# prajwaljpj/GUAVA_renderer

Measured on AMD Instinct MI355X. Metric: rendered frames/sec @512x512, ~100k Gaussians, higher is better.
Workload: dtype f32; 1 GPU; guava-avatar-synth-100k-512-deform+raster; pipeline=EHM LBS -> Gaussian assembly -> rasterize, gaussians=100000, channels=32, global_batch=32, parallelism=frame-sharded x1, batches_in_flight=4, placement=shared, exp=exact-poly, colour_accum=f32 mfma (bit-exact)

## Files before the change

### guava_renderer_amd/csrc/deform.hip

```cpp
#include <climits>
#include <cstdlib>
#include <string>

#include "../../include/gsr.h"
#include "../../include/gsr_deform.h"
#include "deform_internal.h"
#include "gsr_internal.h"
#include "preprocess_dev.h"

namespace gsr {

#ifndef GSR_DEFORM_NOSTORE
#define GSR_DEFORM_NOSTORE 0
#endif

constexpr int kLbsFrames = 16;
constexpr int kLbsSplit = 4;
constexpr int kLbsSplit1 = 16;

struct Parents {
    int8_t p[GSR_LBS_MAX_JOINTS];
};

__device__ __forceinline__ void rodrigues_one(const float* __restrict__ pose, int t, int pose2rot, float (&R)[9]) {
// ... 275 lines not shown
    if (NB > 0) blend_tiled_mfma_part(as, betas, NB, sd_tiled, NB, t, bA, bok, w, hi, lane, NW);
    if (NP > 0 && v_posed) blend_tiled_mfma_part(ap, feat, NP, pd_tiled, NP, t, bA, bok, w, hi, lane, NW);
#pragma unroll
    for (int r = 0; r < 16; r++) {
        red[w][0][r][lane] = as[r];
        red[w][1][r][lane] = ap[r];
    }
    __syncthreads();
#pragma unroll
    for (int i = 0; i < 16 / NW; i++) {
        const int r = (16 / NW) * w + i;
        const int b = b0 + (r & 3) + 8 * (r >> 2) + 4 * hi;
        if (!mok || b >= B) continue;
        float S = red[0][0][r][lane], Pz = red[0][1][r][lane];
#pragma unroll
        for (int u = 1; u < NW; u++) { S += red[u][0][r][lane]; Pz += red[u][1][r][lane]; }
        const float tv = vt[(int64_t)b * vt_stride + m];
        const float vs = NB > 0 ? tv + S : tv;
        v_shaped[(int64_t)b * M + m] = vs;
        if (v_posed) v_posed[(int64_t)b * M + m] = Pz + vs;
    }
}

__device__ __forceinline__ float blend_tiled_one(const float* __restrict__ coef, const float4* __restrict__ tb,
                                                 int K, int t, int w, int hi, int lane) {
    const int nkg = (K + 7) / 8;
    const float4* __restrict__ p = tb + (int64_t)t * nkg * 64 + lane;
    float acc = 0.f;
    for (int g0 = w; g0 < nkg; g0 += 4 * kTiledUnroll) {
        float4 v[kTiledUnroll];
        float a[kTiledUnroll][4];
#pragma unroll
        for (int u = 0; u < kTiledUnroll; u++) {
            const int g = g0 + 4 * u;
            v[u] = g < nkg ? p[(int64_t)g * 64] : make_float4(0.f, 0.f, 0.f, 0.f);
#pragma unroll
            for (int j = 0; j < 4; j++) {
                const int k = 8 * g + 4 * hi + j;
                a[u][j] = k < K ? coef[k] : 0.f;
            }
        }
#pragma unroll
        for (int u = 0; u < kTiledUnroll; u++) {
            acc = fmaf(a[u][0], v[u].x, acc);
            acc = fmaf(a[u][1], v[u].y, acc);
            acc = fmaf(a[u][2], v[u].z, acc);
// ... 64 lines not shown
static void lbs_blend_attr(size_t lds) {
    static size_t attr = 0;
    if (lds > 65536 && attr < lds) {
        attr = lds;
        hipFuncSetAttribute((const void*)k_lbs_blend<kLbsFrames, kLbsSplit>,
                            hipFuncAttributeMaxDynamicSharedMemorySize, (int)lds);
        hipFuncSetAttribute((const void*)k_lbs_blend<1, kLbsSplit1>, hipFuncAttributeMaxDynamicSharedMemorySize,
                            (int)lds);
    }
}

Blend1Job blend1_job(int M, int NB, int NP, const float* vt, const float* betas, const float* feat, float* vs,
                     float* vp, const GsrLbsSparse* sp, const float* pose, int pose2rot) {
    return Blend1Job{M, NB, vp ? NP : 0, pose2rot, vt, betas, reinterpret_cast<const float4*>(sp->shapedirs_tiled),
                     feat, reinterpret_cast<const float4*>(sp->posedirs_tiled), vs, vp, pose};
}

bool blend_tiled1_applies(int B, int NB, int NP, const float* vp, const GsrLbsSparse* sp) {
    static const bool tiled_on = tune_env("GSR_BLEND_TILED", 1) != 0;
    return B == 1 && tiled_on && sp && (NB == 0 || sp->shapedirs_tiled) && (NP == 0 || !vp || sp->posedirs_tiled) &&
           (NB > 0 || (NP > 0 && vp));
}

static void launch_blend(int B, int M, int NB, int NP, const float* vt, int64_t vt_stride, const float* betas,
                         const float* sd_t, const float* feat, const float* pd, float* vs, float* vp,
                         hipStream_t s, const GsrLbsSparse* sp, const float* pose, int pose2rot) {
    static const bool valu_only = tune_env("GSR_BLEND_VALU", 0) == 1;
    static const bool tiled_on = tune_env("GSR_BLEND_TILED", 1) != 0;
    const bool tiled = tiled_on && sp && (NB == 0 || sp->shapedirs_tiled) &&
                       (NP == 0 || !vp || sp->posedirs_tiled) && (NB > 0 || (NP > 0 && vp));
    if (tiled && B > kLbsFrames && !valu_only) {
        static const int nw_env = tune_env("GSR_BLEND_NW", 0);
        const dim3 grid((M + 31) / 32, (B + 31) / 32);
        const int nw = nw_env == 4 || nw_env == 8 ? nw_env : (grid.x * grid.y <= 512 ? 8 : 4);
        const float4* sdt = reinterpret_cast<const float4*>(sp->shapedirs_tiled);
        const float4* pdt = reinterpret_cast<const float4*>(sp->posedirs_tiled);
        if (nw == 8)
            hipLaunchKernelGGL(k_lbs_blend_tiled<8>, grid, dim3(512), 0, s, B, M, NB, vp ? NP : 0, vt, vt_stride,
                               betas, sdt, feat, pdt, vs, vp);
        else
            hipLaunchKernelGGL(k_lbs_blend_tiled<4>, grid, dim3(256), 0, s, B, M, NB, vp ? NP : 0, vt, vt_stride,
                               betas, sdt, feat, pdt, vs, vp);
        return;
    }
    if (tiled && B == 1) {
        const Blend1Job j = blend1_job(M, NB, NP, vt, betas, feat, vs, vp, sp, pose, pose2rot);
        hipLaunchKernelGGL(k_lbs_blend_tiled1, dim3((M + 31) / 32), dim3(256), 0, s, j);
        return;
    }
    if (B > kLbsFrames && !valu_only) {
        hipLaunchKernelGGL(k_lbs_blend_mfma, dim3((M + 31) / 32, (B + 31) / 32), dim3(256), 0, s, B, M, NB,
                           vp ? NP : 0, vt, vt_stride, betas, sd_t, feat, pd, vs, vp);
        return;
    }
    static const bool single = tune_env("GSR_BLEND_SINGLE", 1) != 0;
    if (B == 1 && single) {
        const size_t lds = lbs_blend_lds(NB, vp ? NP : 0, 1, kLbsSplit1);
// ... 86 lines not shown
        x = fmaf(wv, vs[3 * v], x);
        y = fmaf(wv, vs[3 * v + 1], y);
        z = fmaf(wv, vs[3 * v + 2], z);
    }
#pragma unroll
    for (int off = 32; off > 0; off >>= 1) {
        x += __shfl_xor(x, off);
        y += __shfl_xor(y, off);
        z += __shfl_xor(z, off);
    }
    if (lane < 3) {
        float v = lane == 0 ? x : lane == 1 ? y : z;
        if (joff) v = v + joff[((int64_t)b * J + j) * 3 + lane];
        joints[((int64_t)b * J + j) * 3 + lane] = v;
    }
}

struct ChainJoints {
    const int32_t* row;
    const int32_t* col;
    const float* val;
    const float* vs;
    const float* joff;
};
__global__ __launch_bounds__(16 * GSR_LBS_MAX_JOINTS) void k_lbs_chain(int J, Parents par,
                                                                     const float* __restrict__ rot,
                                                                     float* __restrict__ joints,
                                                                     float* __restrict__ jtrans,
                                                                     float* __restrict__ A,
                                                                     const float* __restrict__ pose, int pose2rot,
                                                                     ChainJoints cj) {
    __shared__ float tm[GSR_LBS_MAX_JOINTS][16];
    __shared__ float ch[GSR_LBS_MAX_JOINTS][16];
    __shared__ int depth[GSR_LBS_MAX_JOINTS];
    __shared__ float sjt[GSR_LBS_MAX_JOINTS * 3];
    __shared__ int maxd;
    const int b = blockIdx.x, t = threadIdx.x;
    const float* Jb = joints + (int64_t)b * J * 3;
    if (cj.row) {
        const int w = t >> 6, lane = t & 63;
        for (int j = w; j < J; j += 16) {
            float x = 0.f, y = 0.f, z = 0.f;
            for (int k = cj.row[j] + lane; k < cj.row[j + 1]; k += 64) {
                const int v = cj.col[k];
                const float wv = cj.val[k];
                x = fmaf(wv, cj.vs[3 * v], x);
                y = fmaf(wv, cj.vs[3 * v + 1], y);
                z = fmaf(wv, cj.vs[3 * v + 2], z);
            }
#pragma unroll
            for (int off = 32; off > 0; off >>= 1) {
                x += __shfl_xor(x, off);
                y += __shfl_xor(y, off);
                z += __shfl_xor(z, off);
            }
            if (lane < 3) {
                float v = lane == 0 ? x : lane == 1 ? y : z;
                if (cj.joff) v = v + cj.joff[j * 3 + lane];
                sjt[3 * j + lane] = v;
                joints[j * 3 + lane] = v;
            }
        }
        __syncthreads();
        Jb = sjt;
    }
    if (t == 0) maxd = 0;
    if (t < J) {
        float R[9];
        if (rot) {
#pragma unroll
            for (int e = 0; e < 9; e++) R[e] = rot[((int64_t)b * J + t) * 9 + e];
        } else {
            rodrigues_one(pose, b * J + t, pose2rot, R);
        }
        float rel[3];
        for (int c = 0; c < 3; c++) rel[c] = t == 0 ? Jb[c] : Jb[3 * t + c] - Jb[3 * par.p[t] + c];
        for (int r = 0; r < 3; r++) {
            for (int c = 0; c < 3; c++) tm[t][4 * r + c] = R[3 * r + c];
            tm[t][4 * r + 3] = rel[r];
        }
        tm[t][12] = 0.f; tm[t][13] = 0.f; tm[t][14] = 0.f; tm[t][15] = 1.f;
        int dd = 0;
        for (int i = t; i > 0 && dd < GSR_LBS_MAX_JOINTS; i = par.p[i]) dd++;
        depth[t] = dd;
    }
// ... 398 lines not shown
        return v >= 1 && v <= 64 ? v : 1;
    }();
    hipLaunchKernelGGL(k_deform_preprocess, dim3(d.nblk, (d.B + fpw - 1) / fpw), dim3(256), 0, s, fpw, dg, d, in,
                       g, o);
}

struct PackTable {
    GsrRowSegment seg[GSR_PACK_MAX_SEGMENTS];
};

__global__ __launch_bounds__(256) void k_pack_rows(PackTable t) {
    const GsrRowSegment sg = t.seg[blockIdx.x];
    const int b = blockIdx.y;
    for (int c = threadIdx.x; c < sg.width; c += 256)
        sg.dst[b * sg.dst_stride + c] = sg.src ? sg.src[b * sg.src_stride + c] : 0.f;
}

namespace {

size_t align256(size_t x) { return (x + 255) & ~(size_t)255; }

struct LbsArena {
    float *rot, *feat, *vs, *vp, *joints, *A;
};

size_t carve_lbs(char* base, int B, int V, int J, LbsArena* a) {
    size_t off = 0;
    auto take = [&](size_t bytes) {
        char* p = base ? base + off : nullptr;
        off += align256(bytes);
        return reinterpret_cast<float*>(p);
    };
    const size_t f = sizeof(float);
    LbsArena t;
    t.rot = take(f * (size_t)B * J * 9);
    t.feat = take(f * (size_t)B * (J > 1 ? J - 1 : 1) * 9);
    t.vs = take(f * (size_t)B * V * 3);
    t.vp = take(f * (size_t)B * V * 3);
    t.joints = take(f * (size_t)B * J * 3);
    t.A = take(f * (size_t)B * J * 16);
    if (a) *a = t;
    return off;
}

int hip_check(const char* what) {
    hipError_t e = hipGetLastError();
    if (e != hipSuccess) return api_fail(GSR_ERR_HIP, (std::string(what) + ": " + hipGetErrorString(e)).c_str());
    return 0;
}

}
}

using namespace gsr;

__global__ __launch_bounds__(256) void k_lbs_tile_base(int K, int M, int64_t n4, const float* __restrict__ base,
                                                       float4* __restrict__ tiled) {
    const int64_t i = (int64_t)blockIdx.x * 256 + threadIdx.x;
    if (i >= n4) return;
    const int nkg = (K + 7) / 8;
    const int lane = (int)(i & 63);
    const int64_t tg = i >> 6;
    const int g = (int)(tg % nkg), t = (int)(tg / nkg);
    const int m = 32 * t + (lane & 31), k0 = 8 * g + 4 * (lane >> 5);
    float v[4];
#pragma unroll
    for (int j = 0; j < 4; j++) v[j] = (m < M && k0 + j < K) ? base[(int64_t)(k0 + j) * M + m] : 0.f;
    tiled[i] = make_float4(v[0], v[1], v[2], v[3]);
}

extern "C" {

size_t gsr_lbs_workspace_bytes(int B, int V, int J, int NB) {
    (void)NB;
    if (B <= 0 || V <= 0 || J <= 0) return 0;
    return carve_lbs(nullptr, B, V, J, nullptr);
}

}

namespace {
void launch_joints(int B, int V, int J, const float* J_regressor, const GsrLbsSparse* sp, const float* vs,
                   const float* joints_offset, float* joints, hipStream_t s) {
    if (sp && sp->jreg_row) {
        hipLaunchKernelGGL(k_lbs_joints_csr, dim3((B * J + 3) / 4), dim3(256), 0, s, B, V, J, sp->jreg_row,
                           sp->jreg_col, sp->jreg_val, vs, joints_offset, joints);
    } else {
        hipLaunchKernelGGL(k_lbs_joints, dim3((J + kJointsPerWG - 1) / kJointsPerWG, B), dim3(256), 0, s, V, J,
                           J_regressor, vs, joints_offset, joints);
    }
}
int check_sparse(const GsrLbsSparse* sp, int J, int NB, int V, const char* who) {
    if (!sp) return 0;
    if (sp->jreg_row && (!sp->jreg_col || !sp->jreg_val))
        return api_fail(GSR_ERR_ARG, (std::string(who) + ": jreg_row without jreg_col / jreg_val").c_str());
    if (sp->skin_k && (sp->skin_k < 0 || sp->skin_k > GSR_LBS_SKIN_MAX_K || !sp->skin_joint || !sp->skin_weight))
        return api_fail(GSR_ERR_ARG, (std::string(who) + ": skin_k must be in [1, 16] with its arrays").c_str());
    if (((uintptr_t)sp->shapedirs_tiled | (uintptr_t)sp->posedirs_tiled) & 15)
        return api_fail(GSR_ERR_ARG, (std::string(who) + ": tiled bases must be 16-byte aligned").c_str());
// ... 10 lines not shown
int gsr_lbs(int B, int V, int J, int NB, const float* v_template, int64_t v_template_stride,
            const float* betas, const float* shapedirs_t, const float* pose, int pose2rot,
            const float* posedirs, const float* J_regressor, const int32_t* parents_host,
            const float* lbs_weights_t, const float* joints_offset, float* verts,
            float* joints_transformed, float* joints, float* vert_transforms,
            float* joint_transforms, float* v_shaped, char* workspace, void* stream) {
    return gsr_lbs_sp(B, V, J, NB, v_template, v_template_stride, betas, shapedirs_t, pose, pose2rot, posedirs,
                      J_regressor, parents_host, lbs_weights_t, joints_offset, verts, joints_transformed, joints,
                      vert_transforms, joint_transforms, v_shaped, workspace, nullptr, stream);
}

int gsr_lbs_sp(int B, int V, int J, int NB, const float* v_template, int64_t v_template_stride,
               const float* betas, const float* shapedirs_t, const float* pose, int pose2rot,
               const float* posedirs, const float* J_regressor, const int32_t* parents_host,
               const float* lbs_weights_t, const float* joints_offset, float* verts,
               float* joints_transformed, float* joints, float* vert_transforms,
               float* joint_transforms, float* v_shaped, char* workspace, const GsrLbsSparse* sp,
               void* stream) {
    return gsr::lbs_run(B, V, J, NB, v_template, v_template_stride, betas, shapedirs_t, pose, pose2rot, posedirs,
                        J_regressor, parents_host, lbs_weights_t, joints_offset, verts, joints_transformed, joints,
                        vert_transforms, joint_transforms, v_shaped, workspace, sp, stream, true);
}

}

int gsr::lbs_run(int B, int V, int J, int NB, const float* v_template, int64_t v_template_stride,
                 const float* betas, const float* shapedirs_t, const float* pose, int pose2rot,
                 const float* posedirs, const float* J_regressor, const int32_t* parents_host,
                 const float* lbs_weights_t, const float* joints_offset, float* verts,
                 float* joints_transformed, float* joints, float* vert_transforms,
                 float* joint_transforms, float* v_shaped, char* workspace, const GsrLbsSparse* sp,
                 void* stream, bool skin, const Blend1Job* companion, bool* companion_done) {
    if (companion_done) *companion_done = false;
    if (B <= 0 || V <= 0) return api_fail(GSR_ERR_ARG, "gsr_lbs: B and V must be positive");
    if (int rc = check_sparse(sp, J, betas ? NB : 0, V, "gsr_lbs")) return rc;
    if (J < 1 || J > GSR_LBS_MAX_JOINTS) return api_fail(GSR_ERR_ARG, "gsr_lbs: J must be in [1, 64]");
    if (!v_template || !pose || !J_regressor || !parents_host || !lbs_weights_t || (skin && !verts) || !workspace)
        return api_fail(GSR_ERR_ARG, "gsr_lbs: null required pointer");
    if (J > 1 && !posedirs) return api_fail(GSR_ERR_ARG, "gsr_lbs: posedirs is null");
    if (v_template_stride != 0 && v_template_stride != (int64_t)V * 3)
        return api_fail(GSR_ERR_ARG, "gsr_lbs: v_template stride must be 0 or V*3");
    if (betas) {
        if (NB <= 0 || !shapedirs_t) return api_fail(GSR_ERR_ARG, "gsr_lbs: betas need NB > 0 and shapedirs");
    } else {
        NB = 0;
    }
    Parents par;
    for (int i = 0; i < GSR_LBS_MAX_JOINTS; i++) par.p[i] = -1;
    if (parents_host[0] != -1) return api_fail(GSR_ERR_ARG, "gsr_lbs: parents[0] must be -1");
    for (int i = 1; i < J; i++) {
        if (parents_host[i] < 0 || parents_host[i] >= i)
            return api_fail(GSR_ERR_ARG, "gsr_lbs: parents must satisfy 0 <= parents[i] < i");
        par.p[i] = (int8_t)parents_host[i];
    }
    hipStream_t s = (hipStream_t)stream;
    LbsArena a;
    carve_lbs(workspace, B, V, J, &a);
    float* vs = v_shaped ? v_shaped : a.vs;
    float* jr = joints ? joints : a.joints;
    float* A = joint_transforms ? joint_transforms : a.A;
    const int NP = (J - 1) * 9;
    const int M = V * 3;

    if (lbs_blend_lds(NB, NP, kLbsFrames, kLbsSplit) > 160 * 1024) return api_fail(GSR_ERR_ARG, "gsr_lbs: NB + 9(J-1) too large for LDS");
    const bool fused = blend_takes_pose(B, NB, NP, a.vp, sp);
    if (!fused) {
        hipLaunchKernelGGL(k_lbs_rodrigues, dim3((B * J + 255) / 256), dim3(256), 0, s, B, J, pose,
                           pose2rot, a.rot, a.feat);
        if (int rc = hip_check("lbs_rodrigues")) return rc;
    }
    if (companion && companion_done && blend_tiled1_applies(B, NB, NP, a.vp, sp)) {
        const Blend1Job ja = blend1_job(M, NB, NP, v_template, betas, a.feat, vs, a.vp, sp, fused ? pose : nullptr,
                                        pose2rot);
        const int na = (M + 31) / 32, nb = (companion->M + 31) / 32;
        hipLaunchKernelGGL(k_lbs_blend_tiled1_pair, dim3(na + nb), dim3(256), 0, s, ja, na, *companion);
        *companion_done = true;
    } else {
        launch_blend(B, M, NB, NP, v_template, v_template_stride, betas, shapedirs_t, a.feat, posedirs, vs, a.vp, s,
                     sp, fused ? pose : nullptr, pose2rot);
    }
    if (int rc = hip_check("lbs_blend")) return rc;
    static const bool chain_joints_on = tune_env("GSR_CHAIN_JOINTS", 1) != 0;
    ChainJoints cj{nullptr, nullptr, nullptr, nullptr, nullptr};
    if (B == 1 && sp && sp->jreg_row && chain_joints_on) {
        cj = ChainJoints{sp->jreg_row, sp->jreg_col, sp->jreg_val, vs, joints_offset};
    } else {
        launch_joints(B, V, J, J_regressor, sp, vs, joints_offset, jr, s);
        if (int rc = hip_check("lbs_joints")) return rc;
    }
    hipLaunchKernelGGL(k_lbs_chain, dim3(B), dim3(16 * GSR_LBS_MAX_JOINTS), 0, s, J, par, fused ? nullptr : a.rot,
                       jr, joints_transformed, A, pose, pose2rot, cj);
    if (int rc = hip_check("lbs_chain")) return rc;
    if (!skin) return 0;
    if (sp && sp->skin_k > 0) {
        const dim3 g((V + 255) / 256, B);
        if (sp->skin_k <= 4)
            hipLaunchKernelGGL(k_lbs_skin_ell<4>, g, dim3(256), 0, s, V, J, sp->skin_k, sp->skin_joint,
                               sp->skin_weight, A, a.vp, verts, vert_transforms);
        else if (sp->skin_k <= 8)
            hipLaunchKernelGGL(k_lbs_skin_ell<8>, g, dim3(256), 0, s, V, J, sp->skin_k, sp->skin_joint,
                               sp->skin_weight, A, a.vp, verts, vert_transforms);
        else
            hipLaunchKernelGGL(k_lbs_skin_ell<16>, g, dim3(256), 0, s, V, J, sp->skin_k, sp->skin_joint,
                               sp->skin_weight, A, a.vp, verts, vert_transforms);
    } else {
        hipLaunchKernelGGL(k_lbs_skin, dim3((V + 255) / 256, B), dim3(256), 0, s, V, J, lbs_weights_t, A,
                           a.vp, verts, vert_transforms);
    }
    return hip_check("lbs_skin");
}

template <int KMAX>
__global__ __launch_bounds__(256) void k_skin_splice(int Vh, int Jh, int K, const int32_t* __restrict__ sj,
                                                     const float* __restrict__ sw, const float* __restrict__ A,
                                                     const float* __restrict__ v_posed, int Vb,
                                                     const int32_t* __restrict__ idx,
                                                     const float* __restrict__ r_eyelid,
                                                     const float* __restrict__ l_eyelid,
                                                     const float* __restrict__ eyelid,
                                                     const float* __restrict__ head_scale,
                                                     const float* __restrict__ hjoints, int hj0, int hj1,
                                                     const float* __restrict__ bjoints, int Jb, int bj0, int bj1,
                                                     float* __restrict__ body, uint32_t* __restrict__ bad) {
    __shared__ float As[GSR_LBS_MAX_JOINTS * 16];
    const int b = blockIdx.y;
    for (int i = threadIdx.x; i < Jh * 16; i += blockDim.x) As[i] = A[(int64_t)b * Jh * 16 + i];
    __syncthreads();
    const int v = blockIdx.x * blockDim.x + threadIdx.x;
    if (v >= Vh) return;
    const int d = idx[v];
    if (d < 0 || d >= Vb) {
// ... 26 lines not shown
        float h = T[4 * c] * px + T[4 * c + 1] * py + T[4 * c + 2] * pz + T[4 * c + 3] * 1.0f;
        if (eyelid) {
            h = h + r_eyelid[3 * v + c] * eyelid[2 * b + 1];
            h = h + l_eyelid[3 * v + c] * eyelid[2 * b];
        }
        if (head_scale) h = h * head_scale[3 * b + c];
        float hs = 0.f, bs = 0.f;
        for (int j = hj0; j < hj1; j++) hs += hjb[3 * j + c];
        for (int j = bj0; j < bj1; j++) bs += bjt[3 * j + c];
        body[((int64_t)b * Vb + d) * 3 + c] = (h - hs / (float)(hj1 - hj0)) + bs / (float)(bj1 - bj0);
    }
}

int gsr::lbs_skin_splice(int B, int Vh, int Jh, const GsrLbsSparse* sp_h, const char* ws_h, int Vb,
                         const int32_t* head_index, const float* r_eyelid, const float* l_eyelid,
                         const float* eyelid, const float* head_scale, const float* head_joints, int hj0, int hj1,
                         const float* body_joints, int Jb, int bj0, int bj1, float* body_v_shaped,
                         uint32_t* bad_index_flag, void* stream) {
    if (!sp_h || sp_h->skin_k <= 0) return 1;
    if (hj0 < 0 || hj1 <= hj0 || hj1 > Jh || bj0 < 0 || bj1 <= bj0 || bj1 > Jb)
        return api_fail(GSR_ERR_ARG, "gsr_ehm_forward: bad reference joint ranges");
    if (eyelid && (!r_eyelid || !l_eyelid)) return api_fail(GSR_ERR_ARG, "gsr_ehm_forward: eyelid bases missing");
    LbsArena a;
    carve_lbs(const_cast<char*>(ws_h), B, Vh, Jh, &a);
    const dim3 g((Vh + 255) / 256, B);
    hipStream_t s = (hipStream_t)stream;
#define GSR_SKS(KM)                                                                                              \
    hipLaunchKernelGGL(k_skin_splice<KM>, g, dim3(256), 0, s, Vh, Jh, sp_h->skin_k, sp_h->skin_joint,            \
                       sp_h->skin_weight, a.A, a.vp, Vb, head_index, r_eyelid, l_eyelid, eyelid, head_scale,     \
                       head_joints, hj0, hj1, body_joints, Jb, bj0, bj1, body_v_shaped, bad_index_flag)
    if (sp_h->skin_k <= 4) GSR_SKS(4);
    else if (sp_h->skin_k <= 8) GSR_SKS(8);
    else GSR_SKS(16);
#undef GSR_SKS
    return hip_check("skin_splice");
}

extern "C" {

int gsr_blend_joints(int B, int V, int J, int NB, const float* v_template, int64_t v_template_stride,
                     const float* betas, const float* shapedirs_t, const float* J_regressor,
                     const float* joints_offset, float* v_shaped, float* joints, void* stream) {
    return gsr_blend_joints_sp(B, V, J, NB, v_template, v_template_stride, betas, shapedirs_t, J_regressor,
                               joints_offset, v_shaped, joints, nullptr, stream);
}

int gsr_blend_joints_sp(int B, int V, int J, int NB, const float* v_template, int64_t v_template_stride,
// ... 123 lines not shown
```

### guava_renderer_amd/csrc/deform_internal.h

```cpp
#pragma once
#include <stdint.h>

#include <hip/hip_runtime.h>

#include "../../include/gsr_deform.h"

namespace gsr {
struct Blend1Job {
    int M, NB, NP, pose2rot;
    const float* vt;
    const float* betas;
    const float4* sd_tiled;
    const float* feat;
    const float4* pd_tiled;
    float* v_shaped;
    float* v_posed;
    const float* pose;
};
bool blend_tiled1_applies(int B, int NB, int NP, const float* vp, const GsrLbsSparse* sp);
Blend1Job blend1_job(int M, int NB, int NP, const float* vt, const float* betas, const float* feat, float* vs,
                     float* vp, const GsrLbsSparse* sp, const float* pose, int pose2rot);
int blend_joints_run(int B, int V, int J, int NB, const float* v_template, int64_t v_template_stride,
                     const float* betas, const float* shapedirs_t, const float* J_regressor,
                     const float* joints_offset, float* v_shaped, float* joints, const GsrLbsSparse* sp,
                     void* stream, bool blend_done);
int lbs_run(int B, int V, int J, int NB, const float* v_template, int64_t v_template_stride, const float* betas,
            const float* shapedirs_t, const float* pose, int pose2rot, const float* posedirs,
            const float* J_regressor, const int32_t* parents_host, const float* lbs_weights_t,
            const float* joints_offset, float* verts, float* joints_transformed, float* joints,
            float* vert_transforms, float* joint_transforms, float* v_shaped, char* workspace,
            const GsrLbsSparse* sp, void* stream, bool skin, const Blend1Job* companion = nullptr,
            bool* companion_done = nullptr);
int lbs_skin_splice(int B, int Vh, int Jh, const GsrLbsSparse* sp_h, const char* ws_h, int Vb,
                    const int32_t* head_index, const float* r_eyelid, const float* l_eyelid, const float* eyelid,
                    const float* head_scale, const float* head_joints, int hj0, int hj1, const float* body_joints,
                    int Jb, int bj0, int bj1, float* body_v_shaped, uint32_t* bad_index_flag, void* stream);
}
```

### guava_renderer_amd/csrc/ehm.hip

```cpp
#include <algorithm>
#include <string>
#include <vector>

#include "../../include/gsr.h"
#include "../../include/gsr_deform.h"
#include "deform_internal.h"
#include "gsr_internal.h"

namespace gsr {
namespace {

constexpr int kEhmMaxSegments = 24;
struct EhmPackTable {
    GsrRowSegment seg[kEhmMaxSegments];
};

__global__ __launch_bounds__(256) void k_ehm_pack(EhmPackTable t) {
    const GsrRowSegment sg = t.seg[blockIdx.x];
    const int b = blockIdx.y;
    for (int c = threadIdx.x; c < sg.width; c += 256)
        sg.dst[b * sg.dst_stride + c] = sg.src ? sg.src[b * sg.src_stride + c] : 0.f;
}

size_t al(size_t x) { return (x + 255) & ~(size_t)255; }

struct EhmArena {
    float *betas_h, *pose_h, *betas_b, *pose_b, *hscale, *eyelid, *joff;
    float *hv, *hj, *vt, *tj;
    char *ws_h, *ws_b;
};

size_t carve_ehm(char* base, const GsrEhm& e, int B, EhmArena* a) {
    size_t off = 0;
    auto take = [&](size_t bytes) {
        char* p = base ? base + off : nullptr;
        off += al(bytes);
        return p;
    };
    auto tf = [&](size_t n) { return reinterpret_cast<float*>(take(sizeof(float) * n)); };
    const size_t b = (size_t)B;
    EhmArena t;
    t.betas_h = tf(b * e.flame.NB);
    t.pose_h = tf(b * 3 * e.flame.J);
    t.betas_b = tf(b * e.body.NB);
    t.pose_b = tf(b * 3 * e.body.J);
    t.hscale = tf(b * 3);
    t.eyelid = tf(b * 2);
    t.joff = tf(b * 3 * e.body.J);
    t.hv = tf(b * e.flame.V * 3);
    t.hj = tf(b * e.flame.J * 3);
    t.vt = tf(b * e.body.V * 3);
    t.tj = tf(b * e.body.J * 3);
    t.ws_h = take(gsr_lbs_workspace_bytes(B, e.flame.V, e.flame.J, e.flame.NB));
    t.ws_b = take(gsr_lbs_workspace_bytes(B, e.body.V, e.body.J, 0));
    if (a) *a = t;
    return off;
}

struct Copy {
    int col, width;
    const float* src;
    int64_t src_stride;
};
int add_block(std::vector<GsrRowSegment>& tab, float* dst, int width, std::vector<Copy> cp, const char* what) {
    std::sort(cp.begin(), cp.end(), [](const Copy& x, const Copy& y) { return x.col < y.col; });
    int c = 0;
    for (const Copy& k : cp) {
        if (k.width <= 0) continue;
        if (k.col < c || k.col + k.width > width)
            return api_fail(GSR_ERR_ARG, (std::string("gsr_ehm_forward: ") + what +
                                          ": a parameter does not fit its coefficient columns").c_str());
        if (k.col > c) tab.push_back(GsrRowSegment{nullptr, dst + c, 0, width, k.col - c, 0});
        tab.push_back(GsrRowSegment{k.src, dst + k.col, k.src_stride, width, k.width, 0});
        c = k.col + k.width;
    }
    if (c < width) tab.push_back(GsrRowSegment{nullptr, dst + c, 0, width, width - c, 0});
    return 0;
// ... 89 lines not shown
    }
    const float* hscale = hsc.p;
    if (hsc.p && !direct(hsc)) {
        tab.push_back(GsrRowSegment{hsc.p, a.hscale, hsc.row_stride, 3, 3, 0});
        hscale = a.hscale;
    }
    const float* joff = jof.p;
    if (jof.p && !direct(jof)) {
        tab.push_back(GsrRowSegment{jof.p, a.joff, jof.row_stride, 3 * Jb, 3 * Jb, 0});
        joff = a.joff;
    }
    if (tab.size() > (size_t)kEhmMaxSegments)
        return api_fail(GSR_ERR_ARG, "gsr_ehm_forward: too many coefficient segments");
    EhmPackTable t;
    for (size_t i = 0; i < tab.size(); i++) {
        if (tab[i].width > 4096) return api_fail(GSR_ERR_ARG, "gsr_ehm_forward: coefficient row too wide");
        t.seg[i] = tab[i];
    }
    hipStream_t s = (hipStream_t)stream;
    hipLaunchKernelGGL(k_ehm_pack, dim3((unsigned)tab.size(), B), dim3(256), 0, s, t);
    if (hipError_t err = hipGetLastError(); err != hipSuccess)
        return api_fail(GSR_ERR_HIP, (std::string("ehm_pack: ") + hipGetErrorString(err)).c_str());

    static const bool skin_splice_on = tune_env("GSR_EHM_SKIN_SPLICE", 1) != 0;
    const bool fuse = skin_splice_on && e.flame.sparse && e.flame.sparse->skin_k > 0;
    Blend1Job body_shape{};
    static const bool pair_on = tune_env("GSR_EHM_PAIR", 1) != 0;
    const bool pair = pair_on && B == 1 && blend_tiled1_applies(1, NBb, 0, nullptr, e.body.sparse);
    if (pair)
        body_shape = blend1_job(Vb * 3, NBb, 0, e.body.v_template, a.betas_b, nullptr, a.vt, nullptr, e.body.sparse,
                                nullptr, 1);
    bool body_blended = false;
    int rc = lbs_run(B, Vh, Jh, NBh, e.flame.v_template, 0, a.betas_h, e.flame.shapedirs_t, a.pose_h, 1,
                     e.flame.posedirs, e.flame.J_regressor, e.flame.parents_host, e.flame.lbs_weights_t, nullptr,
                     a.hv, a.hj, nullptr, nullptr, nullptr, nullptr, a.ws_h, e.flame.sparse, stream, !fuse,
                     pair ? &body_shape : nullptr, &body_blended);
    if (rc) return rc;
    rc = blend_joints_run(B, Vb, Jb, NBb, e.body.v_template, 0, a.betas_b, e.body.shapedirs_t, e.body.J_regressor,
                          joff, a.vt, a.tj, e.body.sparse, stream, body_blended);
    if (rc) return rc;
    if (fuse)
        rc = lbs_skin_splice(B, Vh, Jh, e.flame.sparse, a.ws_h, Vb, e.head_index, e.r_eyelid, e.l_eyelid, eyelid,
                             hscale, a.hj, e.hj0, e.hj1, a.tj, Jb, e.bj0, e.bj1, a.vt, e.bad_index_flag, stream);
    else
        rc = gsr_splice_head(B, Vb, Vh, e.head_index, a.hv, e.r_eyelid, e.l_eyelid, eyelid, hscale, a.hj, Jh, e.hj0,
                             e.hj1, a.tj, Jb, e.bj0, e.bj1, a.vt, e.bad_index_flag, stream);
// ... 9 lines not shown
```

Baseline: 17360 frames/s.

## Add batched EHM path with pre-tiled coefficient MFMA blend and paired launches

Adds a batched EHM forward path for B>16 that pre-tiles betas and pose features into MFMA-ready layouts in a single kernel. Head and body shape blends then run in one paired MFMA launch, and the head chain is merged with body joint regression in one launch. The aim is fewer kernel launches and removing the per-block coefficient staging from the blend kernels. It costs extra workspace and a larger code path with new tiled buffers.

After: 17640 frames/s (median of 6 runs). 1.6% higher.

```diff
diff --git a/guava_renderer_amd/csrc/deform.hip b/guava_renderer_amd/csrc/deform.hip
--- a/guava_renderer_amd/csrc/deform.hip
+++ b/guava_renderer_amd/csrc/deform.hip
@@ -321,6 +321,140 @@
     }
 }
 
+__device__ __forceinline__ int64_t coef_tile_index(int nkg, int b, int k) {
+    return ((((int64_t)(b >> 5) * nkg + (k >> 3)) * 64 + 32 * ((k >> 2) & 1) + (b & 31)) << 2) + (k & 3);
+}
+
+struct CoefJob {
+    int B, J, NB, pose2rot;
+    int n_pose, n_beta;
+    const float* pose;
+    const float* betas;
+    float* feat_tiles;
+    float4* beta_tiles;
+};
+
+__device__ __forceinline__ void coef_tiles_one(const CoefJob& c, int idx) {
+    if (idx < c.n_pose) {
+        const int J = c.J, NP = 9 * (J - 1), nkg = (NP + 7) / 8;
+        const int b = idx / J, j = idx - b * J;
+        float R[9];
+        if (b < c.B) {
+            rodrigues_one(c.pose, idx, c.pose2rot, R);
+#pragma unroll
+            for (int e = 0; e < 9; e++) R[e] = R[e] - ((e % 4) == 0 ? 1.0f : 0.0f);
+        } else {
+#pragma unroll
+            for (int e = 0; e < 9; e++) R[e] = 0.f;
+        }
+        if (j > 0) {
+#pragma unroll
+            for (int e = 0; e < 9; e++) c.feat_tiles[coef_tile_index(nkg, b, 9 * (j - 1) + e)] = R[e];
+            if (j == J - 1)
+                for (int k = NP; k < 8 * nkg; k++) c.feat_tiles[coef_tile_index(nkg, b, k)] = 0.f;
+        }
+        return;
+    }
+    idx -= c.n_pose;
+    if (idx >= c.n_beta) return;
+    const int NB = c.NB, nkg = (NB + 7) / 8;
+    const int lane = idx & 63, tg = idx >> 6;
+    const int g = tg % nkg, bt = tg / nkg;
+    const int b = 32 * bt + (lane & 31), k0 = 8 * g + 4 * (lane >> 5);
+    float v[4];
+#pragma unroll
+    for (int j = 0; j < 4; j++) v[j] = (b < c.B && k0 + j < NB) ? c.betas[(int64_t)b * NB + k0 + j] : 0.f;
+    c.beta_tiles[idx] = make_float4(v[0], v[1], v[2], v[3]);
+}
+
+__global__ __launch_bounds__(256) void k_lbs_coef_tiles(CoefJob a, CoefJob b) {
+    const int i = blockIdx.x * 256 + threadIdx.x;
+    const int na = a.n_pose + a.n_beta;
+    if (i < na) coef_tiles_one(a, i);
+    else if (i - na < b.n_pose + b.n_beta) coef_tiles_one(b, i - na);
+}
+
+__device__ __forceinline__ void blend_tiledc_mfma_part(floatx16& acc, const float4* __restrict__ ct,
+                                                       const float4* __restrict__ tb, int K, int t, int bt, int w,
+                                                       int lane, int nw) {
+    const int nkg = (K + 7) / 8;
+    const float4* __restrict__ p = tb + (int64_t)t * nkg * 64 + lane;
+    const float4* __restrict__ c = ct + (int64_t)bt * nkg * 64 + lane;
+    auto mma = [&](const float4& v, const float4& a) {
+        acc = __builtin_amdgcn_mfma_f32_32x32x2f32(a.x, v.x, acc, 0, 0, 0);
+        acc = __builtin_amdgcn_mfma_f32_32x32x2f32(a.y, v.y, acc, 0, 0, 0);
+        acc = __builtin_amdgcn_mfma_f32_32x32x2f32(a.z, v.z, acc, 0, 0, 0);
+        acc = __builtin_amdgcn_mfma_f32_32x32x2f32(a.w, v.w, acc, 0, 0, 0);
+    };
+    if (w >= nkg) return;
+    float4 v0 = p[(int64_t)w * 64], a0 = c[(int64_t)w * 64], v1, a1;
+    for (int g = w; g < nkg; g += 2 * nw) {
+        const bool more = g + nw < nkg;
+        if (more) { v1 = p[(int64_t)(g + nw) * 64]; a1 = c[(int64_t)(g + nw) * 64]; }
+        mma(v0, a0);
+        if (more) {
+            if (g + 2 * nw < nkg) { v0 = p[(int64_t)(g + 2 * nw) * 64]; a0 = c[(int64_t)(g + 2 * nw) * 64]; }
+            mma(v1, a1);
+        }
+    }
+}
+
+struct BlendTJob {
+    int M, NB, NP;
+    const float* vt;
+    int64_t vt_stride;
+    const float4* beta_tiles;
+    const float4* sd_tiled;
+    const float4* feat_tiles;
+    const float4* pd_tiled;
+    float* v_shaped;
+    float* v_posed;
+};
+
+template <int WAVES, int KS>
+__device__ __forceinline__ void blend_tiledc_block(const BlendTJob& j, int B, int tw, int bt,
+                                                   float (*red)[2][16][64]) {
+    const int lane = threadIdx.x & 63, w8 = threadIdx.x >> 6, hi = lane >> 5, l32 = lane & 31;
+    const int sg = w8 / KS, w = w8 % KS;
+    const int M = j.M, NB = j.NB;
+    const int t = tw * (WAVES / KS) + sg;
+    const bool tok = t < (M + 31) / 32;
+    const int m = t * 32 + l32, b0 = bt * 32;
+    const bool mok = tok && m < M;
+    floatx16 as, ap;
+#pragma unroll
+    for (int r = 0; r < 16; r++) { as[r] = 0.f; ap[r] = 0.f; }
+    if (tok && NB > 0) blend_tiledc_mfma_part(as, j.beta_tiles, j.sd_tiled, NB, t, bt, w, lane, KS);
+    if (tok && j.NP > 0 && j.v_posed)
+        blend_tiledc_mfma_part(ap, j.feat_tiles, j.pd_tiled, j.NP, t, bt, w, lane, KS);
+#pragma unroll
+    for (int r = 0; r < 16; r++) {
+        red[w8][0][r][lane] = as[r];
+        red[w8][1][r][lane] = ap[r];
+    }
+    __syncthreads();
+#pragma unroll
+    for (int i = 0; i < 16 / KS; i++) {
+        const int r = (16 / KS) * w + i;
+        const int b = b0 + (r & 3) + 8 * (r >> 2) + 4 * hi;
+        if (!mok || b >= B) continue;
+        float S = red[sg * KS][0][r][lane], Pz = red[sg * KS][1][r][lane];
+#pragma unroll
+        for (int u = 1; u < KS; u++) { S += red[sg * KS + u][0][r][lane]; Pz += red[sg * KS + u][1][r][lane]; }
+        const float tv = j.vt[(int64_t)b * j.vt_stride + m];
+        const float vs = NB > 0 ? tv + S : tv;
+        j.v_shaped[(int64_t)b * M + m] = vs;
+        if (j.v_posed) j.v_posed[(int64_t)b * M + m] = Pz + vs;
+    }
+}
+
+template <int WAVES, int KSA, int KSB>
+__global__ __launch_bounds__(64 * WAVES) void k_lbs_blend_tiledc(int B, BlendTJob a, int na, BlendTJob b) {
+    __shared__ float red[WAVES][2][16][64];
+    if ((int)blockIdx.x < na) blend_tiledc_block<WAVES, KSA>(a, B, blockIdx.x, blockIdx.y, red);
+    else blend_tiledc_block<WAVES, KSB>(b, B, blockIdx.x - na, blockIdx.y, red);
+}
+
 __device__ __forceinline__ float blend_tiled_one(const float* __restrict__ coef, const float4* __restrict__ tb,
                                                  int K, int t, int w, int hi, int lane) {
     const int nkg = (K + 7) / 8;
@@ -431,6 +565,11 @@
            (NB > 0 || (NP > 0 && vp));
 }
 
+static int blend_ksplit(int M) {
+    static const int nw_env = tune_env("GSR_BLEND_NW", 0);
+    return nw_env == 4 || nw_env == 8 ? nw_env : ((M + 31) / 32 <= 512 ? 8 : 4);
+}
+
 static void launch_blend(int B, int M, int NB, int NP, const float* vt, int64_t vt_stride, const float* betas,
                          const float* sd_t, const float* feat, const float* pd, float* vs, float* vp,
                          hipStream_t s, const GsrLbsSparse* sp, const float* pose, int pose2rot) {
@@ -439,9 +578,8 @@
     const bool tiled = tiled_on && sp && (NB == 0 || sp->shapedirs_tiled) &&
                        (NP == 0 || !vp || sp->posedirs_tiled) && (NB > 0 || (NP > 0 && vp));
     if (tiled && B > kLbsFrames && !valu_only) {
-        static const int nw_env = tune_env("GSR_BLEND_NW", 0);
         const dim3 grid((M + 31) / 32, (B + 31) / 32);
-        const int nw = nw_env == 4 || nw_env == 8 ? nw_env : (grid.x * grid.y <= 512 ? 8 : 4);
+        const int nw = blend_ksplit(M);
         const float4* sdt = reinterpret_cast<const float4*>(sp->shapedirs_tiled);
         const float4* pdt = reinterpret_cast<const float4*>(sp->posedirs_tiled);
         if (nw == 8)
@@ -574,45 +712,55 @@
     const float* val;
     const float* vs;
     const float* joff;
+    float* joints;
+    int V, J;
 };
+__device__ __forceinline__ void chain_regress_joints(const ChainJoints& cj, int b, int t, float* sjt) {
+    const int w = t >> 6, lane = t & 63;
+    const float* vs = cj.vs + (int64_t)b * cj.V * 3;
+    for (int j = w; j < cj.J; j += 16) {
+        float x = 0.f, y = 0.f, z = 0.f;
+        for (int k = cj.row[j] + lane; k < cj.row[j + 1]; k += 64) {
+            const int v = cj.col[k];
+            const float wv = cj.val[k];
+            x = fmaf(wv, vs[3 * v], x);
+            y = fmaf(wv, vs[3 * v + 1], y);
+            z = fmaf(wv, vs[3 * v + 2], z);
+        }
+#pragma unroll
+        for (int off = 32; off > 0; off >>= 1) {
+            x += __shfl_xor(x, off);
+            y += __shfl_xor(y, off);
+            z += __shfl_xor(z, off);
+        }
+        if (lane < 3) {
+            float v = lane == 0 ? x : lane == 1 ? y : z;
+            if (cj.joff) v = v + cj.joff[((int64_t)b * cj.J + j) * 3 + lane];
+            if (sjt) sjt[3 * j + lane] = v;
+            cj.joints[((int64_t)b * cj.J + j) * 3 + lane] = v;
+        }
+    }
+}
 __global__ __launch_bounds__(16 * GSR_LBS_MAX_JOINTS) void k_lbs_chain(int J, Parents par,
                                                                      const float* __restrict__ rot,
-                                                                     float* __restrict__ joints,
+                                                                     const float* __restrict__ joints,
                                                                      float* __restrict__ jtrans,
                                                                      float* __restrict__ A,
                                                                      const float* __restrict__ pose, int pose2rot,
-                                                                     ChainJoints cj) {
+                                                                     ChainJoints cj, int nchain, ChainJoints xj) {
     __shared__ float tm[GSR_LBS_MAX_JOINTS][16];
     __shared__ float ch[GSR_LBS_MAX_JOINTS][16];
     __shared__ int depth[GSR_LBS_MAX_JOINTS];
     __shared__ float sjt[GSR_LBS_MAX_JOINTS * 3];
     __shared__ int maxd;
     const int b = blockIdx.x, t = threadIdx.x;
+    if (b >= nchain) {
+        chain_regress_joints(xj, b - nchain, t, nullptr);
+        return;
+    }
     const float* Jb = joints + (int64_t)b * J * 3;
     if (cj.row) {
-        const int w = t >> 6, lane = t & 63;
-        for (int j = w; j < J; j += 16) {
-            float x = 0.f, y = 0.f, z = 0.f;
-            for (int k = cj.row[j] + lane; k < cj.row[j + 1]; k += 64) {
-                const int v = cj.col[k];
-                const float wv = cj.val[k];
-                x = fmaf(wv, cj.vs[3 * v], x);
-                y = fmaf(wv, cj.vs[3 * v + 1], y);
-                z = fmaf(wv, cj.vs[3 * v + 2], z);
-            }
-#pragma unroll
-            for (int off = 32; off > 0; off >>= 1) {
-                x += __shfl_xor(x, off);
-                y += __shfl_xor(y, off);
-                z += __shfl_xor(z, off);
-            }
-            if (lane < 3) {
-                float v = lane == 0 ? x : lane == 1 ? y : z;
-                if (cj.joff) v = v + cj.joff[j * 3 + lane];
-                sjt[3 * j + lane] = v;
-                joints[j * 3 + lane] = v;
-            }
-        }
+        chain_regress_joints(cj, b, t, sjt);
         __syncthreads();
         Jb = sjt;
     }
@@ -1057,9 +1205,12 @@
 
 struct LbsArena {
     float *rot, *feat, *vs, *vp, *joints, *A;
+    float *beta_tiles, *feat_tiles;
 };
 
-size_t carve_lbs(char* base, int B, int V, int J, LbsArena* a) {
+size_t coef_tile_floats(int B, int K) { return (size_t)((B + 31) / 32) * (size_t)((K + 7) / 8) * 256; }
+
+size_t carve_lbs(char* base, int B, int V, int J, int NB, LbsArena* a) {
     size_t off = 0;
     auto take = [&](size_t bytes) {
         char* p = base ? base + off : nullptr;
@@ -1074,6 +1225,8 @@
     t.vp = take(f * (size_t)B * V * 3);
     t.joints = take(f * (size_t)B * J * 3);
     t.A = take(f * (size_t)B * J * 16);
+    t.beta_tiles = take(f * coef_tile_floats(B, NB > 0 ? NB : 0));
+    t.feat_tiles = take(f * coef_tile_floats(B, 9 * (J - 1)));
     if (a) *a = t;
     return off;
 }
@@ -1107,9 +1260,8 @@
 extern "C" {
 
 size_t gsr_lbs_workspace_bytes(int B, int V, int J, int NB) {
-    (void)NB;
     if (B <= 0 || V <= 0 || J <= 0) return 0;
-    return carve_lbs(nullptr, B, V, J, nullptr);
+    return carve_lbs(nullptr, B, V, J, NB, nullptr);
 }
 
 }
@@ -1166,6 +1318,88 @@
                         vert_transforms, joint_transforms, v_shaped, workspace, sp, stream, true);
 }
 
+}
+
+namespace gsr {
+namespace {
+bool blend_tiledc_applies(int B, int NB, int NP, const float* vp, const GsrLbsSparse* sp) {
+    static const bool on = tune_env("GSR_BLEND_TILED", 1) != 0 && tune_env("GSR_BLEND_VALU", 0) != 1 &&
+                           tune_env("GSR_BLEND_COEF_TILES", 1) != 0;
+    return on && B > kLbsFrames && sp && (NB == 0 || sp->shapedirs_tiled) &&
+           (NP == 0 || !vp || sp->posedirs_tiled) && (NB > 0 || (NP > 0 && vp));
+}
+
+CoefJob coef_job(int B, int J, int NB, const float* pose, int pose2rot, const float* betas, const LbsArena& a,
+                 float* beta_tiles) {
+    CoefJob c{};
+    c.B = B; c.J = J; c.NB = betas ? NB : 0; c.pose2rot = pose2rot;
+    c.n_pose = (pose && J > 1) ? (B + 31) / 32 * 32 * J : 0;
+    c.n_beta = c.NB > 0 ? (int)(coef_tile_floats(B, c.NB) / 4) : 0;
+    c.pose = pose; c.betas = betas;
+    c.feat_tiles = a.feat_tiles;
+    c.beta_tiles = reinterpret_cast<float4*>(beta_tiles);
+    return c;
+}
+
+void launch_coef_tiles(const CoefJob& a, const CoefJob& b, hipStream_t s) {
+    const int n = a.n_pose + a.n_beta + b.n_pose + b.n_beta;
+    if (n == 0) return;
+    hipLaunchKernelGGL(k_lbs_coef_tiles, dim3((n + 255) / 256), dim3(256), 0, s, a, b);
+}
+
+BlendTJob blendt_job(int M, int NB, int NP, const float* vt, int64_t vt_stride, const float* beta_tiles,
+                     const float* feat_tiles, float* vs, float* vp, const GsrLbsSparse* sp) {
+    return BlendTJob{M, NB, vp ? NP : 0, vt, vt_stride, reinterpret_cast<const float4*>(beta_tiles),
+                     reinterpret_cast<const float4*>(sp->shapedirs_tiled), reinterpret_cast<const float4*>(feat_tiles),
+                     reinterpret_cast<const float4*>(sp->posedirs_tiled), vs, vp};
+}
+
+void launch_blend_tiledc(int B, const BlendTJob& a, const BlendTJob* b, hipStream_t s) {
+    const int ka = blend_ksplit(a.M), kb = b ? blend_ksplit(b->M) : ka;
+    const int waves = ka > kb ? ka : kb;
+    const int na = ((a.M + 31) / 32 + waves / ka - 1) / (waves / ka);
+    const int nb = b ? ((b->M + 31) / 32 + waves / kb - 1) / (waves / kb) : 0;
+    const dim3 grid(na + nb, (B + 31) / 32);
+    const BlendTJob jb = b ? *b : a;
+#define GSR_BTC(W, KA, KB) \
+    hipLaunchKernelGGL((k_lbs_blend_tiledc<W, KA, KB>), grid, dim3(64 * W), 0, s, B, a, na, jb)
+    if (ka == 4 && kb == 4) GSR_BTC(4, 4, 4);
+    else if (ka == 8 && kb == 8) GSR_BTC(8, 8, 8);
+    else if (ka == 8) GSR_BTC(8, 8, 4);
+    else GSR_BTC(8, 4, 8);
+#undef GSR_BTC
+}
+
+int make_parents(int J, const int32_t* parents_host, Parents* par) {
+    for (int i = 0; i < GSR_LBS_MAX_JOINTS; i++) par->p[i] = -1;
+    if (parents_host[0] != -1) return api_fail(GSR_ERR_ARG, "gsr_lbs: parents[0] must be -1");
+    for (int i = 1; i < J; i++) {
+        if (parents_host[i] < 0 || parents_host[i] >= i)
+            return api_fail(GSR_ERR_ARG, "gsr_lbs: parents must satisfy 0 <= parents[i] < i");
+        par->p[i] = (int8_t)parents_host[i];
+    }
+    return 0;
+}
+
+void launch_skin(int B, int V, int J, const float* lbs_weights_t, const GsrLbsSparse* sp, const float* A,
+                 const float* vp, float* verts, float* vert_transforms, hipStream_t s) {
+    if (sp && sp->skin_k > 0) {
+        const dim3 g((V + 255) / 256, B);
+        if (sp->skin_k <= 4)
+            hipLaunchKernelGGL(k_lbs_skin_ell<4>, g, dim3(256), 0, s, V, J, sp->skin_k, sp->skin_joint,
+                               sp->skin_weight, A, vp, verts, vert_transforms);
+        else if (sp->skin_k <= 8)
+            hipLaunchKernelGGL(k_lbs_skin_ell<8>, g, dim3(256), 0, s, V, J, sp->skin_k, sp->skin_joint,
+                               sp->skin_weight, A, vp, verts, vert_transforms);
+        else
+            hipLaunchKernelGGL(k_lbs_skin_ell<16>, g, dim3(256), 0, s, V, J, sp->skin_k, sp->skin_joint,
+                               sp->skin_weight, A, vp, verts, vert_transforms);
+    } else {
+        hipLaunchKernelGGL(k_lbs_skin, dim3((V + 255) / 256, B), dim3(256), 0, s, V, J, lbs_weights_t, A, vp, verts,
+                           vert_transforms);
+    }
+}
+}
 }
 
 int gsr::lbs_run(int B, int V, int J, int NB, const float* v_template, int64_t v_template_stride,
@@ -1190,16 +1424,10 @@
         NB = 0;
     }
     Parents par;
-    for (int i = 0; i < GSR_LBS_MAX_JOINTS; i++) par.p[i] = -1;
-    if (parents_host[0] != -1) return api_fail(GSR_ERR_ARG, "gsr_lbs: parents[0] must be -1");
-    for (int i = 1; i < J; i++) {
-        if (parents_host[i] < 0 || parents_host[i] >= i)
-            return api_fail(GSR_ERR_ARG, "gsr_lbs: parents must satisfy 0 <= parents[i] < i");
-        par.p[i] = (int8_t)parents_host[i];
-    }
+    if (int rc = make_parents(J, parents_host, &par)) return rc;
     hipStream_t s = (hipStream_t)stream;
     LbsArena a;
-    carve_lbs(workspace, B, V, J, &a);
+    carve_lbs(workspace, B, V, J, NB, &a);
     float* vs = v_shaped ? v_shaped : a.vs;
     float* jr = joints ? joints : a.joints;
     float* A = joint_transforms ? joint_transforms : a.A;
@@ -1208,12 +1436,19 @@
 
     if (lbs_blend_lds(NB, NP, kLbsFrames, kLbsSplit) > 160 * 1024) return api_fail(GSR_ERR_ARG, "gsr_lbs: NB + 9(J-1) too large for LDS");
     const bool fused = blend_takes_pose(B, NB, NP, a.vp, sp);
-    if (!fused) {
+    const bool tilec = blend_tiledc_applies(B, NB, NP, a.vp, sp);
+    if (tilec) {
+        launch_coef_tiles(coef_job(B, J, NB, pose, pose2rot, betas, a, a.beta_tiles), CoefJob{}, s);
+        if (int rc = hip_check("lbs_coef_tiles")) return rc;
+    } else if (!fused) {
         hipLaunchKernelGGL(k_lbs_rodrigues, dim3((B * J + 255) / 256), dim3(256), 0, s, B, J, pose,
                            pose2rot, a.rot, a.feat);
         if (int rc = hip_check("lbs_rodrigues")) return rc;
     }
-    if (companion && companion_done && blend_tiled1_applies(B, NB, NP, a.vp, sp)) {
+    if (tilec) {
+        const BlendTJob j = blendt_job(M, NB, NP, v_template, v_template_stride, a.beta_tiles, a.feat_tiles, vs, a.vp, sp);
+        launch_blend_tiledc(B, j, nullptr, s);
+    } else if (companion && companion_done && blend_tiled1_applies(B, NB, NP, a.vp, sp)) {
         const Blend1Job ja = blend1_job(M, NB, NP, v_template, betas, a.feat, vs, a.vp, sp, fused ? pose : nullptr,
                                         pose2rot);
         const int na = (M + 31) / 32, nb = (companion->M + 31) / 32;
@@ -1225,32 +1460,91 @@
     }
     if (int rc = hip_check("lbs_blend")) return rc;
     static const bool chain_joints_on = tune_env("GSR_CHAIN_JOINTS", 1) != 0;
-    ChainJoints cj{nullptr, nullptr, nullptr, nullptr, nullptr};
-    if (B == 1 && sp && sp->jreg_row && chain_joints_on) {
-        cj = ChainJoints{sp->jreg_row, sp->jreg_col, sp->jreg_val, vs, joints_offset};
+    static const bool chain_batch_on = tune_env("GSR_CHAIN_BATCH", 1) != 0;
+    ChainJoints cj{};
+    if ((B == 1 || (tilec && chain_batch_on)) && sp && sp->jreg_row && chain_joints_on) {
+        cj = ChainJoints{sp->jreg_row, sp->jreg_col, sp->jreg_val, vs, joints_offset, jr, V, J};
     } else {
         launch_joints(B, V, J, J_regressor, sp, vs, joints_offset, jr, s);
         if (int rc = hip_check("lbs_joints")) return rc;
     }
-    hipLaunchKernelGGL(k_lbs_chain, dim3(B), dim3(16 * GSR_LBS_MAX_JOINTS), 0, s, J, par, fused ? nullptr : a.rot,
-                       jr, joints_transformed, A, pose, pose2rot, cj);
+    hipLaunchKernelGGL(k_lbs_chain, dim3(B), dim3(16 * GSR_LBS_MAX_JOINTS), 0, s, J, par,
+                       (fused || tilec) ? nullptr : a.rot, jr, joints_transformed, A, pose, pose2rot, cj, B,
+                       ChainJoints{});
     if (int rc = hip_check("lbs_chain")) return rc;
     if (!skin) return 0;
-    if (sp && sp->skin_k > 0) {
-        const dim3 g((V + 255) / 256, B);
-        if (sp->skin_k <= 4)
-            hipLaunchKernelGGL(k_lbs_skin_ell<4>, g, dim3(256), 0, s, V, J, sp->skin_k, sp->skin_joint,
-                               sp->skin_weight, A, a.vp, verts, vert_transforms);
-        else if (sp->skin_k <= 8)
-            hipLaunchKernelGGL(k_lbs_skin_ell<8>, g, dim3(256), 0, s, V, J, sp->skin_k, sp->skin_joint,
-                               sp->skin_weight, A, a.vp, verts, vert_transforms);
-        else
-            hipLaunchKernelGGL(k_lbs_skin_ell<16>, g, dim3(256), 0, s, V, J, sp->skin_k, sp->skin_joint,
-                               sp->skin_weight, A, a.vp, verts, vert_transforms);
+    launch_skin(B, V, J, lbs_weights_t, sp, A, a.vp, verts, vert_transforms, s);
+    return hip_check("lbs_skin");
+}
+
+bool gsr::ehm_batch_applies(int B, const GsrLbsSparse* sp_h, const GsrLbsSparse* sp_b, int NBh, int NBb) {
+    static const bool on = tune_env("GSR_EHM_BATCH", 1) != 0 && tune_env("GSR_CHAIN_JOINTS", 1) != 0 &&
+                           tune_env("GSR_CHAIN_BATCH", 1) != 0 && tune_env("GSR_EHM_SKIN_SPLICE", 1) != 0;
+    if (!on || !sp_h || !sp_b || NBh <= 0 || NBb <= 0) return false;
+    auto ok = [&](const GsrLbsSparse* sp, int NB) {
+        return sp->jreg_row && sp->skin_k > 0 && sp->shapedirs_tiled && sp->posedirs_tiled &&
+               blend_tiledc_applies(B, NB, 0, nullptr, sp);
+    };
+    return ok(sp_h, NBh) && ok(sp_b, NBb);
+}
+
+size_t gsr::lbs_coef_tile_bytes(int B, int K) { return sizeof(float) * coef_tile_floats(B, K); }
+
+int gsr::ehm_batch_run(int B, const EhmBatchModel& head, const EhmBatchModel& body, float* body_betas_tiles,
+                       float* head_joints_t, float* body_vt, float* body_tj, const float* joints_offset,
+                       const int32_t* head_index, const float* r_eyelid, const float* l_eyelid,
+                       const float* eyelid, const float* head_scale, int hj0, int hj1, int bj0, int bj1,
+                       uint32_t* bad_index_flag, float* verts, float* joints_transformed, float* joints,
+                       float* vert_transforms, float* joint_transforms, void* stream) {
+    const int Vh = head.V, Jh = head.J, Vb = body.V, Jb = body.J;
+    if (int rc = check_sparse(head.sp, Jh, head.NB, Vh, "gsr_ehm_forward")) return rc;
+    if (int rc = check_sparse(body.sp, Jb, body.NB, Vb, "gsr_ehm_forward")) return rc;
+    if (hj0 < 0 || hj1 <= hj0 || hj1 > Jh || bj0 < 0 || bj1 <= bj0 || bj1 > Jb)
+        return api_fail(GSR_ERR_ARG, "gsr_ehm_forward: bad reference joint ranges");
+    if (eyelid && (!r_eyelid || !l_eyelid)) return api_fail(GSR_ERR_ARG, "gsr_ehm_forward: eyelid bases missing");
+    Parents par_h, par_b;
+    if (int rc = make_parents(Jh, head.parents_host, &par_h)) return rc;
+    if (int rc = make_parents(Jb, body.parents_host, &par_b)) return rc;
+    hipStream_t s = (hipStream_t)stream;
+    LbsArena ah, ab;
+    carve_lbs(head.ws, B, Vh, Jh, head.NB, &ah);
+    carve_lbs(body.ws, B, Vb, Jb, 0, &ab);
+    const int NPh = 9 * (Jh - 1), NPb = 9 * (Jb - 1);
+    float* jb = joints ? joints : ab.joints;
+    float* Ab = joint_transforms ? joint_transforms : ab.A;
+    launch_coef_tiles(coef_job(B, Jh, head.NB, head.pose, 1, head.betas, ah, ah.beta_tiles),
+                      coef_job(B, Jb, body.NB, body.pose, 1, body.betas, ab, body_betas_tiles), s);
+    if (int rc = hip_check("ehm_coef_tiles")) return rc;
+    const BlendTJob jh = blendt_job(Vh * 3, head.NB, NPh, head.v_template, head.vt_stride, ah.beta_tiles,
+                                    ah.feat_tiles, ah.vs, ah.vp, head.sp);
+    const BlendTJob jt = blendt_job(Vb * 3, body.NB, 0, body.v_template, body.vt_stride, body_betas_tiles, nullptr,
+                                    body_vt, nullptr, body.sp);
+    static const bool pair_on = tune_env("GSR_EHM_BATCH_PAIR", 1) != 0;
+    if (pair_on) {
+        launch_blend_tiledc(B, jh, &jt, s);
     } else {
-        hipLaunchKernelGGL(k_lbs_skin, dim3((V + 255) / 256, B), dim3(256), 0, s, V, J, lbs_weights_t, A,
-                           a.vp, verts, vert_transforms);
-    }
+        launch_blend_tiledc(B, jh, nullptr, s);
+        launch_blend_tiledc(B, jt, nullptr, s);
+    }
+    if (int rc = hip_check("ehm_blend_pair")) return rc;
+    const ChainJoints cjh{head.sp->jreg_row, head.sp->jreg_col, head.sp->jreg_val, ah.vs, nullptr, ah.joints, Vh, Jh};
+    const ChainJoints cjt{body.sp->jreg_row, body.sp->jreg_col, body.sp->jreg_val, body_vt, joints_offset, body_tj,
+                          Vb, Jb};
+    hipLaunchKernelGGL(k_lbs_chain, dim3(2 * B), dim3(16 * GSR_LBS_MAX_JOINTS), 0, s, Jh, par_h, nullptr, ah.joints,
+                       head_joints_t, ah.A, head.pose, 1, cjh, B, cjt);
+    if (int rc = hip_check("ehm_head_chain")) return rc;
+    if (int rc = lbs_skin_splice(B, Vh, Jh, head.sp, head.ws, Vb, head_index, r_eyelid, l_eyelid, eyelid, head_scale,
+                                 head_joints_t, hj0, hj1, body_tj, Jb, bj0, bj1, body_vt, bad_index_flag, stream))
+        return rc;
+    const BlendTJob jp = blendt_job(Vb * 3, 0, NPb, body_vt, (int64_t)Vb * 3, nullptr, ab.feat_tiles, ab.vs, ab.vp,
+                                    body.sp);
+    launch_blend_tiledc(B, jp, nullptr, s);
+    if (int rc = hip_check("ehm_body_blend")) return rc;
+    const ChainJoints cjb{body.sp->jreg_row, body.sp->jreg_col, body.sp->jreg_val, ab.vs, joints_offset, jb, Vb, Jb};
+    hipLaunchKernelGGL(k_lbs_chain, dim3(B), dim3(16 * GSR_LBS_MAX_JOINTS), 0, s, Jb, par_b, nullptr, jb,
+                       joints_transformed, Ab, body.pose, 1, cjb, B, ChainJoints{});
+    if (int rc = hip_check("ehm_body_chain")) return rc;
+    launch_skin(B, Vb, Jb, nullptr, body.sp, Ab, ab.vp, verts, vert_transforms, s);
     return hip_check("lbs_skin");
 }
 
@@ -1323,7 +1617,7 @@
         return api_fail(GSR_ERR_ARG, "gsr_ehm_forward: bad reference joint ranges");
     if (eyelid && (!r_eyelid || !l_eyelid)) return api_fail(GSR_ERR_ARG, "gsr_ehm_forward: eyelid bases missing");
     LbsArena a;
-    carve_lbs(const_cast<char*>(ws_h), B, Vh, Jh, &a);
+    carve_lbs(const_cast<char*>(ws_h), B, Vh, Jh, 0, &a);
     const dim3 g((Vh + 255) / 256, B);
     hipStream_t s = (hipStream_t)stream;
 #define GSR_SKS(KM)                                                                                              \
diff --git a/guava_renderer_amd/csrc/deform_internal.h b/guava_renderer_amd/csrc/deform_internal.h
--- a/guava_renderer_amd/csrc/deform_internal.h
+++ b/guava_renderer_amd/csrc/deform_internal.h
@@ -20,6 +20,24 @@
 bool blend_tiled1_applies(int B, int NB, int NP, const float* vp, const GsrLbsSparse* sp);
 Blend1Job blend1_job(int M, int NB, int NP, const float* vt, const float* betas, const float* feat, float* vs,
                      float* vp, const GsrLbsSparse* sp, const float* pose, int pose2rot);
+struct EhmBatchModel {
+    int V, J, NB;
+    const float* v_template;
+    int64_t vt_stride;
+    const float* betas;
+    const float* pose;
+    const int32_t* parents_host;
+    const GsrLbsSparse* sp;
+    char* ws;
+};
+bool ehm_batch_applies(int B, const GsrLbsSparse* sp_h, const GsrLbsSparse* sp_b, int NBh, int NBb);
+int ehm_batch_run(int B, const EhmBatchModel& head, const EhmBatchModel& body, float* body_betas_tiles,
+                  float* head_joints_t, float* body_vt, float* body_tj, const float* joints_offset,
+                  const int32_t* head_index, const float* r_eyelid, const float* l_eyelid, const float* eyelid,
+                  const float* head_scale, int hj0, int hj1, int bj0, int bj1, uint32_t* bad_index_flag,
+                  float* verts, float* joints_transformed, float* joints, float* vert_transforms,
+                  float* joint_transforms, void* stream);
+size_t lbs_coef_tile_bytes(int B, int K);
 int blend_joints_run(int B, int V, int J, int NB, const float* v_template, int64_t v_template_stride,
                      const float* betas, const float* shapedirs_t, const float* J_regressor,
                      const float* joints_offset, float* v_shaped, float* joints, const GsrLbsSparse* sp,
diff --git a/guava_renderer_amd/csrc/ehm.hip b/guava_renderer_amd/csrc/ehm.hip
--- a/guava_renderer_amd/csrc/ehm.hip
+++ b/guava_renderer_amd/csrc/ehm.hip
@@ -28,6 +28,7 @@
     float *betas_h, *pose_h, *betas_b, *pose_b, *hscale, *eyelid, *joff;
     float *hv, *hj, *vt, *tj;
     char *ws_h, *ws_b;
+    float* betas_b_tiles;
 };
 
 size_t carve_ehm(char* base, const GsrEhm& e, int B, EhmArena* a) {
@@ -53,6 +54,7 @@
     t.tj = tf(b * e.body.J * 3);
     t.ws_h = take(gsr_lbs_workspace_bytes(B, e.flame.V, e.flame.J, e.flame.NB));
     t.ws_b = take(gsr_lbs_workspace_bytes(B, e.body.V, e.body.J, 0));
+    t.betas_b_tiles = reinterpret_cast<float*>(take(lbs_coef_tile_bytes(B, e.body.NB)));
     if (a) *a = t;
     return off;
 }
@@ -188,6 +190,16 @@
     if (hipError_t err = hipGetLastError(); err != hipSuccess)
         return api_fail(GSR_ERR_HIP, (std::string("ehm_pack: ") + hipGetErrorString(err)).c_str());
 
+    if (ehm_batch_applies(B, e.flame.sparse, e.body.sparse, NBh, NBb)) {
+        const EhmBatchModel mh{Vh, Jh, NBh, e.flame.v_template, 0, a.betas_h, a.pose_h, e.flame.parents_host,
+                               e.flame.sparse, a.ws_h};
+        const EhmBatchModel mb{Vb, Jb, NBb, e.body.v_template, 0, a.betas_b, a.pose_b, e.body.parents_host,
+                               e.body.sparse, a.ws_b};
+        return ehm_batch_run(B, mh, mb, a.betas_b_tiles, a.hj, a.vt, a.tj, joff, e.head_index, e.r_eyelid,
+                             e.l_eyelid, eyelid, hscale, e.hj0, e.hj1, e.bj0, e.bj1, e.bad_index_flag, out->vertices,
+                             out->joints_transform, out->joints, out->ver_transform_mat, out->joint_transform_mat,
+                             stream);
+    }
     static const bool skin_splice_on = tune_env("GSR_EHM_SKIN_SPLICE", 1) != 0;
     const bool fuse = skin_splice_on && e.flame.sparse && e.flame.sparse->skin_k > 0;
     Blend1Job body_shape{};
```
